# harryjfowen/PointsToWood

Hardware: AMD Instinct MI355X
Metric: classified points/sec (higher is better)
Workload: dtype f16x3

## Files before the change

include/p2w.h:

```cpp
#ifndef P2W_H
#define P2W_H

#include <stddef.h>
#include <stdint.h>

#ifdef __cplusplus
extern "C" {
#endif

typedef void* p2w_stream_t;

#define P2W_OK 0
#define P2W_EINVAL (-1)
#define P2W_ENULL (-2)
#define P2W_EALIGN (-3)
#define P2W_EWORKSPACE (-4)
#define P2W_EUNSUPPORTED (-5)

#define P2W_MAX_K 64
#define P2W_MAX_K_WIDE 100
#define P2W_MAX_K_CONV 32

int32_t p2w_version(void);
const char* p2w_strerror(int32_t code);
// ... 190 lines not shown
                    const float* sf, const int32_t* nbr, const int32_t* deg, int32_t kw, int32_t M,
                    const float* w1r4 , const float* W2p, int32_t C1, int32_t C2,
                    const float* b2, const float* bn_s, const float* bn_t, float* out, int32_t ldo,
                    p2w_stream_t stream);

#define P2W_PREC_F16X3 0
#define P2W_PREC_F16 1
#define P2W_PREC_BF16 2
int32_t p2w_packed_dims_h(int32_t prec, int32_t N, int32_t K, int32_t* N_pad, int32_t* K_pad);

#define P2W_GEMM_TILE_128 1
#define P2W_GEMM_TILE_256 2
#define P2W_GEMM_GENERIC_EPI 4
#define P2W_GEMM_ORDER_ROWS 8
#define P2W_GEMM_ORDER_COLS 16
#define P2W_GEMM_RESIDUAL_H 32
#define P2W_GEMM_STREAMK 64
#define P2W_GEMM_NO_STREAMK 128
#define P2W_GEMM_TILE_64 (1 << 24)
#define P2W_GEMM_NO_TILE_64 (1 << 25)
#define P2W_SA_ITEM_256 1
#define P2W_SA_ITEM_128 2
#define P2W_SA_PACK8 4

int32_t p2w_gemm_h2(int32_t prec, const void* A_h, int32_t ldh_a, const void* Wh, float wscale, int32_t M, int32_t N,
                    int32_t K, const p2w_epilogue* epi, float* out_f32, int32_t ldo, void* out_h, int32_t ldh_o,
                    int32_t flags, p2w_stream_t stream);
size_t p2w_gemm_h2_sk_ws_bytes(void);
int32_t p2w_gemm_h2_sk(int32_t prec, const void* A_h, int32_t ldh_a, const void* Wh, float wscale, int32_t M, int32_t N,
                       int32_t K, const p2w_epilogue* epi, float* out_f32, int32_t ldo, void* out_h, int32_t ldh_o,
                       void* ws, size_t ws_bytes, int32_t flags, p2w_stream_t stream);
size_t p2w_gemm_h2_rowdot_ws_bytes(int32_t M, int32_t N);
int32_t p2w_gemm_h2_rowdot(int32_t prec, const void* A_h, int32_t ldh_a, const void* Wh, float wscale, int32_t M, int32_t N,
                           int32_t K, const p2w_epilogue* epi, const float* dot_w, float dot_b, float* out, void* ws,
                           size_t ws_bytes, int32_t flags, p2w_stream_t stream);
size_t p2w_sa_conv_h_ws_bytes(int32_t M, int32_t flags);
int32_t p2w_sa_conv_h(int32_t prec, const float* P, int32_t ldp, int32_t n_src, const float* xyzr_src, const int32_t* idx,
                      const int32_t* batch_dst, const float* sf, const int32_t* nbr, const int32_t* deg, int32_t kw,
                      int32_t M, const float* w1r4, const void* W2h, float wscale, int32_t C1, int32_t C2,
                      const float* b2, const float* bn_s, const float* bn_t, float* out, int32_t ldo, void* out_h,
                      int32_t ldh, void* ws, size_t ws_bytes, int32_t flags, p2w_stream_t stream);
int32_t p2w_sa_conv_h_rows(int32_t prec, const float* P, int32_t ldp, int32_t n_src, const float* xyzr_src, const int32_t* idx,
                           const int32_t* batch_dst, const float* sf, const int32_t* nbr, const int32_t* deg, int32_t kw,
                           int32_t M, const float* w1r4, const void* W2h, float wscale, int32_t C1, int32_t C2,
                           const float* b2, const float* bn_s, const float* bn_t, float* out, int32_t ldo, void* out_h,
                           int32_t ldh, void* ws, size_t ws_bytes, int32_t flags, const int32_t* src_row, uint32_t* range,
// ... 132 lines not shown
```

pointstowood_amd/_lib.py:

```python
from __future__ import annotations

import ctypes as C
import os

import torch

_HERE = os.path.dirname(os.path.abspath(__file__))
LIB_PATH = os.path.join(_HERE, "libp2w_gfx950.so")

_vp, _i32, _f32, _sz = C.c_void_p, C.c_int32, C.c_float, C.c_size_t


class Epilogue(C.Structure):
    _fields_ = [("bias", _vp), ("sc0", _vp), ("sh0", _vp), ("sc1", _vp), ("sh1", _vp), ("residual", _vp),
                ("ldr", _i32), ("relu0", _i32), ("relu1", _i32), ("relu2", _i32), ("relu_final", _i32), ("range", _vp),
                ("interp", _vp), ("interp_rows", _i32)]


class BnStage(C.Structure):
    _fields_ = [("dw_w", _vp), ("dw_b", _vp), ("gamma", _vp), ("beta", _vp), ("running_mean", _vp), ("running_var", _vp),
                ("momentum", C.c_double), ("eps", C.c_double), ("relu", _i32)]


SEARCH_X_INDEX_IN_W, SEARCH_Q_ROW_IN_W, SEARCH_BOX = 1, 2, 4
PREC_F16X3, PREC_F16, PREC_BF16 = 0, 1, 2
PREC_OF = {"f16x3": PREC_F16X3, "fp16": PREC_F16, "bf16": PREC_BF16}
GEMM_TILE_128, GEMM_TILE_256, GEMM_GENERIC_EPI, GEMM_ORDER_ROWS, GEMM_ORDER_COLS, GEMM_RESIDUAL_H = 1, 2, 4, 8, 16, 32
GEMM_STREAMK, GEMM_NO_STREAMK = 64, 128
SA_ITEM_256, SA_ITEM_128, SA_PACK8 = 1, 2, 4
CLUSTER_LINK, CLUSTER_COMPRESS, CLUSTER_NUMBER, CLUSTER_ALL = 1, 2, 4, 7
MAX_K_WIDE = 100
EVAL_CHUNK, EVAL_MAX_CLASSES = 4096, 8
LOSS_CHUNK = 4096
EDGE_CHUNK = 1024
BN_GROUP = 16
BN_CHAIN_MAX, BN_CHAIN_ROWS = 3, 32
FEED_CHUNK, FEED_STREAM = 256, 0x50325746
SAMPLE_STREAM, SAMPLE_TILE, SAMPLE_N_MAX = 0x50325753, 1024, 1 << 24
F32, F16 = 0, 1

SIGNATURES = {
    "p2w_version": (_i32, []),
    "p2w_strerror": (C.c_char_p, [_i32]),
    "p2w_pack_xyzr": (_i32, [_vp, _i32, _vp, _vp, _i32, _i32, _vp, _vp, _vp]),
    "p2w_voxel_sample_ws_bytes": (_sz, [_i32]),
    "p2w_voxel_sample": (_i32, [_vp, _vp, _i32, _i32, _f32, _vp, _vp, _vp, _vp, _vp, _vp, _vp, _vp, _vp, _vp, _sz, _vp]),
    "p2w_voxel_sample_table_ws_bytes": (_sz, [_i32, C.c_int64]),
    "p2w_voxel_sample_table": (_i32, [_vp, _vp, _i32, _i32, _f32, _vp, _vp, _vp, _vp, _vp, _vp, _vp, _vp, _vp, _vp, _vp, _vp, C.c_int64,
                                      _vp, _sz, _vp]),
    "p2w_voxel_sample_table_prepare": (_i32, [_vp, _sz, _vp]),
    "p2w_voxel_sample_table_prepared": (_i32, [_vp, _vp, _i32, _i32, _f32, _vp, _vp, _vp, _vp, _vp, _vp, _vp, _vp, _vp, _vp, _vp, _vp, C.c_int64,
                                               _vp, _sz, _vp]),
# ... 189 lines not shown
```

pointstowood_amd/csrc/p2w_feat.hip:

```cpp
#include "p2w_hgemm.h"
#include "p2w_segmax.h"

constexpr int G_BM = 128, G_BN = 128, G_BK = 32, G_LD = 36;

extern "C" void p2w_packed_dims(int32_t N, int32_t K, int32_t* N_pad, int32_t* K_pad) {
    if (N_pad) *N_pad = (N + 255) / 256 * 256;
    if (K_pad) *K_pad = (K + G_BK - 1) / G_BK * G_BK;
}
extern "C" int32_t p2w_packed_dims_h(int32_t prec, int32_t N, int32_t K, int32_t* N_pad, int32_t* K_pad) {
    if (prec < P2W_PREC_F16X3 || prec > P2W_PREC_BF16) return P2W_EINVAL;
    const int ka = prec == P2W_PREC_F16X3 ? 32 : 64;
    if (N_pad) *N_pad = (N + 255) / 256 * 256;
    if (K_pad) *K_pad = (K + ka - 1) / ka * ka;
    return P2W_OK;
}

__device__ __forceinline__ void mma_slab(const float* __restrict__ As, const float* __restrict__ Bs, int wr, int wc, int lane,
                                         f32x16 (&acc)[2][2]) {
    const int r = lane & 31, h = lane >> 5;
#pragma unroll
    for (int kk = 0; kk < G_BK; kk += 8) {
        const float4 a0 = *reinterpret_cast<const float4*>(&As[(wr * 64 + r) * G_LD + kk + 4 * h]);
        const float4 a1 = *reinterpret_cast<const float4*>(&As[(wr * 64 + 32 + r) * G_LD + kk + 4 * h]);
        const float4 b0 = *reinterpret_cast<const float4*>(&Bs[(wc * 64 + r) * G_LD + kk + 4 * h]);
// ... 364 lines not shown
    EpiArgs ep = {};
    if (epi) {
        if ((epi->sc0 && !epi->sh0) || (epi->sc1 && !epi->sh1)) return P2W_ENULL;
        if (epi->residual || epi->interp) return P2W_EUNSUPPORTED;
        ep = {epi->bias, epi->sc0, epi->sh0, epi->sc1, epi->sh1, nullptr, 0, epi->relu0, epi->relu1, epi->relu2, epi->relu_final, nullptr, epi->range, nullptr};
    }
    const _Float16* Ah = static_cast<const _Float16*>(A_h);
    const _Float16* Wp = static_cast<const _Float16*>(Wh);
    const int ldpart = rowdot_ldpart(M);
    const int32_t rc = prec == P2W_PREC_F16X3
        ? launch_gemm_h<0>(Ah, ldh_a, Wp, wscale, M, N, K, ep, nullptr, 0, nullptr, 0, flags, p2w_s(stream), dot_w, part, ldpart)
        : p2w_gemm_h1_impl(prec, Ah, ldh_a, Wp, wscale, M, N, K, ep, nullptr, 0, nullptr, 0, flags, p2w_s(stream), dot_w, part, ldpart);
    if (rc != P2W_OK) return rc;
    rowdot_finish_kernel<<<p2w_cdiv(M, 256), 256, 0, p2w_s(stream)>>>(part, ldpart, (N + 63) / 64, dot_b, M, out);
    return P2W_LAUNCH_STATUS();
}

__global__ __launch_bounds__(256) void sa_edge_meta_kernel(const float4* __restrict__ xyzr, const int* __restrict__ idx,
                                                           const int* __restrict__ batch_dst, const float* __restrict__ sf,
                                                           const int* __restrict__ nbr, const int* __restrict__ deg, int kw,
                                                           int M, int n_src, int ldp4, int G, const int* __restrict__ list,
                                                           const int* __restrict__ n_list_dev, const int* __restrict__ src_row,
                                                           int* __restrict__ meta_j, float4* __restrict__ meta_g, int* __restrict__ desc,
                                                           float4* __restrict__ zero_row) {
    const long g = (long)blockIdx.x * 256 + threadIdx.x;
    if (zero_row && g < ldp4) zero_row[g] = make_float4(0.f, 0.f, 0.f, 0.f);
    const int n_groups = list ? *n_list_dev : M;
    const int gpt = 32 / G;
    const long n_tiles = ((long)n_groups + gpt - 1) / gpt;
    if (g >= n_tiles * 32) return;
    const int gi = (int)(g / G), slot = (int)(g % G);
    const int tgt = gi < n_groups ? (list ? list[gi] : gi) : -1;
    int j = 0, d = 0;
    float rx = 0.f, ry = 0.f, rz = 0.f, rf = 0.f, nrm = 0.f;
    bool valid = false;
    if (tgt >= 0) {
        d = min(deg[tgt], kw);
        const int self = idx[tgt];
        const float s = sf[batch_dst[tgt]];
        const float4 pi = xyzr[self];
        valid = slot < d;
        j = valid ? nbr[(size_t)tgt * kw + slot] : self;
        if (j < 0) j = self;
        const float4 pj = xyzr[j];
        if (valid) {
            rx = pj.x / s - pi.x / s; ry = pj.y / s - pi.y / s; rz = pj.z / s - pi.z / s;
            nrm = sqrtf(((rx * rx) + (ry * ry)) + (rz * rz));
            rf = pj.w;
        }
    }
    float dmax = nrm;
    for (int off = G >> 1; off >= 1; off >>= 1) dmax = fmaxf(dmax, __shfl_xor(dmax, off));
    const float den = dmax + 1e-8f;
    meta_j[g] = (valid ? (src_row ? src_row[j] : j) : n_src) * ldp4;
    meta_g[g] = make_float4(rx / den, ry / den, rz / den, rf);
    if (slot == 0) desc[gi] = tgt >= 0 ? ((tgt << 6) | d) : -1;
}

__global__ __launch_bounds__(SA_PART_BLOCK) void sa_part_count_kernel(const int* __restrict__ deg, int kw, int M, int* __restrict__ blk_small) {
    const int t = blockIdx.x * SA_PART_BLOCK + threadIdx.x;
    const bool small = t < M && min(deg[t], kw) <= 8;
    const int c = __syncthreads_count(small);
    if (threadIdx.x == 0) blk_small[blockIdx.x] = c;
}
__global__ __launch_bounds__(1024) void sa_part_scan_kernel(int* __restrict__ blk_small, int nblk, int M, int* __restrict__ counts) {
    __shared__ int part[1024];
    const int per = (nblk + 1023) / 1024, b0 = threadIdx.x * per, b1 = min(b0 + per, nblk);
    int sum = 0;
    for (int b = b0; b < b1; ++b) sum += blk_small[b];
    part[threadIdx.x] = sum;
    __syncthreads();
    for (int off = 1; off < 1024; off <<= 1) {
        const int v = threadIdx.x >= off ? part[threadIdx.x - off] : 0;
        __syncthreads();
        part[threadIdx.x] += v;
        __syncthreads();
    }
    int run = part[threadIdx.x] - sum;
// ... 370 lines not shown
```

pointstowood_amd/csrc/p2w_hgemm.h:

```cpp
#pragma once
#include "p2w_common.h"
#include <type_traits>

typedef float f32x16 __attribute__((ext_vector_type(16)));
typedef _Float16 h8 __attribute__((ext_vector_type(8)));
typedef __bf16 bf8 __attribute__((ext_vector_type(8)));
typedef __fp16 hpair __attribute__((ext_vector_type(2)));
typedef _Float16 hpairn __attribute__((ext_vector_type(2)));
typedef __bf16 bpair __attribute__((ext_vector_type(2)));
typedef float fpair __attribute__((ext_vector_type(2)));
typedef __attribute__((address_space(3))) void* lds_vp;
typedef const __attribute__((address_space(1))) void* glb_vp;

constexpr int H_BK = 32;
constexpr int SA_EPI_COLS = 1024;

template <int PREC> struct HCfg {
    static constexpr int planes = PREC == 0 ? 2 : 1;
    static constexpr int kslab = PREC == 0 ? 32 : 64;
    static constexpr int kalign = PREC == 0 ? 32 : 64;
};

template <int PREC>
__device__ __forceinline__ f32x16 h_mfma(h8 a, h8 b, f32x16 c) {
    if constexpr (PREC == 2)
        return __builtin_amdgcn_mfma_f32_32x32x16_bf16(__builtin_bit_cast(bf8, a), __builtin_bit_cast(bf8, b), c, 0, 0, 0);
    else
        return __builtin_amdgcn_mfma_f32_32x32x16_f16(a, b, c, 0, 0, 0);
}

typedef float f32x4 __attribute__((ext_vector_type(4)));
template <int PREC>
__device__ __forceinline__ f32x4 h_mfma16(h8 a, h8 b, f32x4 c) {
    if constexpr (PREC == 2)
        return __builtin_amdgcn_mfma_f32_16x16x32_bf16(__builtin_bit_cast(bf8, a), __builtin_bit_cast(bf8, b), c, 0, 0, 0);
    else
        return __builtin_amdgcn_mfma_f32_16x16x32_f16(a, b, c, 0, 0, 0);
}

__device__ __forceinline__ void split_pair(float a, float b, unsigned& hi, unsigned& lo) {
    const hpair h = __builtin_amdgcn_cvt_pkrtz(a, b);
    const fpair rem = {a - (float)h[0], b - (float)h[1]};
    const hpairn l = __builtin_convertvector(rem, hpairn);
    hi = __builtin_bit_cast(unsigned, h);
    lo = __builtin_bit_cast(unsigned, l);
}
template <int PREC>
__device__ __forceinline__ unsigned pack_pair(float a, float b) {
    if constexpr (PREC == 2) {
        const fpair p = {a, b};
        return __builtin_bit_cast(unsigned, __builtin_convertvector(p, bpair));
    } else {
        const fpair p = {__builtin_amdgcn_fmed3f(a, -65504.f, 65504.f), __builtin_amdgcn_fmed3f(b, -65504.f, 65504.f)};
        return __builtin_bit_cast(unsigned, __builtin_convertvector(p, hpairn));
    }
}
template <int PREC>
__device__ __forceinline__ void h_store2(_Float16* __restrict__ base, unsigned ldh, unsigned row, unsigned col, float a, float b) {
    if constexpr (PREC == 0) {
        unsigned hw, lw;
        split_pair(a, b, hw, lw);
        _Float16* p = base + (size_t)row * (2 * ldh) + 64 * (col >> 5) + (col & 31);
        *reinterpret_cast<unsigned*>(p) = hw;
        *reinterpret_cast<unsigned*>(p + 32) = lw;
    } else {
        *reinterpret_cast<unsigned*>(base + (size_t)row * ldh + col) = pack_pair<PREC>(a, b);
    }
}
// ... 806 lines not shown
#pragma unroll
                    for (int r = 0; r < 4; ++r) {
                        const int slot = r + 4 * h;
                        if (slot < d) ext = fmaxf(ext, sgn * acc[i][j][4 * q + r]);
                    }
                }
                {
                    const auto sw = __builtin_amdgcn_permlane32_swap(__float_as_uint(ext), __float_as_uint(ext), false, false);
                    ext = fmaxf(__uint_as_float(sw[0]), __uint_as_float(sw[1]));
                }
                float vmax = fmaf(fmaxf(fmaf(sgn * ext, wscale, e.bias[j]), 0.f), e.s[j], e.t[j]);
                if (d == 0 || !cv) vmax = 0.f;
                amax = nan_max(amax, fabsf(vmax));
                if (cv && h == 0 && out) out[(size_t)tgt * ldo + col] = vmax;
                if (out_h2) {
                    const float nb = __uint_as_float(__builtin_amdgcn_update_dpp(0, __float_as_uint(vmax), 0xB1, 0xf, 0xf, false));
                    if (h == 0 && (lane & 1) == 0 && col < ldh) h_store2<PREC>(out_h2, ldh, tgt, col, vmax, nb);
                }
            }
        }
    }
}

template <int PREC, int BN, int RT, int G>
__global__ __launch_bounds__(512, 2) void sa_conv16p_kernel(const float* __restrict__ P, int ldp, const int* __restrict__ meta_j,
                                                            const float4* __restrict__ meta_g, const int* __restrict__ desc,
                                                            const int* __restrict__ tiles_dev, int M, const float* __restrict__ w1r4, int C1, int C1pad,
                                                            const _Float16* __restrict__ W2h, size_t plane, float wscale, int C2,
                                                            int nMt_, int nNt, const float* __restrict__ b2,
                                                            const float* __restrict__ bn_s, const float* __restrict__ bn_t,
                                                            float* __restrict__ out, int ldo, _Float16* __restrict__ out_h2,
                                                            int ldh, unsigned* __restrict__ range) {
    constexpr int NP = HCfg<PREC>::planes;
    constexpr int WCn = BN / 64, BM = 32 * RT * (8 / WCn), NW = 8, NR = BM / 128;
    constexpr int GPT = 32 / G;
    if (tiles_dev) M = *tiles_dev;
    const int nMt = tiles_dev ? (M + BM / 32 - 1) / (BM / 32) : nMt_;
    if (M <= 0) return;
    constexpr int A_CH = 4 * NP * BM, STAGE_CH = A_CH + 4 * NP * BN;
    constexpr int NWI = 4;
    constexpr int NI = (4 * NP * BN) / 64 / NWI;
    static_assert(NI >= 1, "every issuing wave has at least one W2 DMA piece per slab");
    __shared__ __attribute__((aligned(16))) char S[2 * STAGE_CH * 16 + 4 * 512 * 4 + 3 * SA_EPI_COLS * 4];
    float* const Wr = reinterpret_cast<float*>(S + 2 * STAGE_CH * 16);
    float* const Ep = Wr + 4 * 512;
    const int tid = threadIdx.x, lane = tid & 63;
    for (int i = tid; i < 4 * C1pad; i += 512) Wr[i] = w1r4[i];
    for (int i = tid; i < C2; i += 512) { Ep[i] = b2[i]; Ep[SA_EPI_COLS + i] = bn_s[i]; Ep[2 * SA_EPI_COLS + i] = bn_t[i]; }
    const int wave = __builtin_amdgcn_readfirstlane(tid >> 6), wr = wave / WCn, wc = wave % WCn;
    const int nitems = nMt * nNt, nslab = C1pad / H_BK;
    int first, stride, limit;
    if ((gridDim.x & 7) == 0) {
        const int xcd = blockIdx.x & 7, slot = blockIdx.x >> 3, per = gridDim.x >> 3;
        const int chunk = (nitems + 7) >> 3;
        first = xcd * chunk + slot; stride = per; limit = min((xcd + 1) * chunk, nitems);
    } else {
        first = blockIdx.x; stride = gridDim.x; limit = nitems;
    }
    if (first >= limit) return;
    const int my_items = (limit - first + stride - 1) / stride;
    const int total = my_items * nslab;

    auto item_mt = [&](int it) { return (first + it * stride) / nNt; };
    auto item_nt = [&](int it) { return (first + it * stride) % nNt; };

    constexpr int RCH = 4 * NP;
    auto img = [](int row, int chunk) { return (row * RCH + (NP == 2 ? (chunk ^ ((row >> 1) & 7)) : (chunk ^ ((row >> 2) & 3)))) * 16; };
    auto imgA = [](int row, int chunk) { return (row * RCH + (NP == 2 ? (chunk ^ ((row >> 1) & 7) ^ ((row & 1) << 2)) : (chunk ^ ((row >> 2) & 3)))) * 16; };
    const int prow = tid >> 2, pq = tid & 3;
    const int a_dst = imgA(prow, pq);
    size_t boff[NI];
    int dstc[NI];
    (void)plane;
#pragma unroll
    for (int i = 0; i < NI; ++i) {
        const int g2 = (wave % NWI) + NWI * i;
        const int row = (NP == 2 ? 8 : 16) * g2 + (lane >> (NP == 2 ? 3 : 2));
        const int c = NP == 2 ? ((lane & 7) ^ ((row >> 1) & 7)) : ((lane & 3) ^ ((row >> 2) & 3));
        boff[i] = (size_t)row * (NP * C1pad) + 8 * c;
        dstc[i] = A_CH + g2 * 64;
    }
    constexpr int KADV = NP == 2 ? 2 : 1;
    auto issue = [&](int stage, const _Float16* wbase, int k0) {
        if (wave >= NWI) return;
#pragma unroll
        for (int i = 0; i < NI; ++i)
            __builtin_amdgcn_global_load_lds((glb_vp)(wbase + boff[i] + KADV * k0),
                                             (lds_vp)(S + ((size_t)stage * STAGE_CH + dstc[i]) * 16), 16, 0, 0);
    };
    struct Meta { int j[NR]; float4 g[NR]; };
    struct Vals { float4 v[NR][2]; };
    const int last_row = M * 32 - 1;
    auto load_meta = [&](int mt_, Meta& m) {
#pragma unroll
        for (int u = 0; u < NR; ++u) {
            const int row = min(mt_ * BM + prow + 128 * u, last_row);
            m.j[u] = meta_j[row];
            m.g[u] = meta_g[row];
        }
    };
    auto gather = [&](const Meta& m, int k0, Vals& dst) {
        const unsigned k4 = (unsigned)(k0 >> 2) + 2u * pq;
#pragma unroll
        for (int u = 0; u < NR; ++u) {
            const float4* p = reinterpret_cast<const float4*>(P) + ((unsigned)m.j[u] + k4);
            dst.v[u][0] = p[0];
            dst.v[u][1] = p[1];
        }
    };
    struct WRegs { float4 w[2][4]; };
    auto load_w = [&](int k0, WRegs& wr_) {
        const int k = k0 + 8 * pq;
#pragma unroll
        for (int half = 0; half < 2; ++half)
#pragma unroll
            for (int c = 0; c < 4; ++c) wr_.w[half][c] = *reinterpret_cast<const float4*>(&Wr[c * C1pad + k + 4 * half]);
    };
    const unsigned lds_base = (unsigned)(uintptr_t)(lds_vp)S;
    auto produce = [&](int stage, const Meta& m, int k0, const Vals& src, const WRegs& wr_) {
        const int k = k0 + 8 * pq;
#pragma unroll
      for (int u = 0; u < NR; ++u) {
        const float4 rg = m.g[u];
        unsigned hiw[4], low[4];
#pragma unroll
        for (int half = 0; half < 2; ++half) {
            const int kk = k + 4 * half;
            const float4 wx = wr_.w[half][0], wy = wr_.w[half][1], wz = wr_.w[half][2], wf = wr_.w[half][3];
            const float4 p = src.v[u][half];
            const float gx = rg.x, gy = rg.y, gz = rg.z, gw = rg.w;
            float v[4];
            v[0] = fmaxf(fmaf(gw, wf.x, fmaf(gz, wz.x, fmaf(gy, wy.x, fmaf(gx, wx.x, p.x)))), 0.f);
            v[1] = fmaxf(fmaf(gw, wf.y, fmaf(gz, wz.y, fmaf(gy, wy.y, fmaf(gx, wx.y, p.y)))), 0.f);
            v[2] = fmaxf(fmaf(gw, wf.z, fmaf(gz, wz.z, fmaf(gy, wy.z, fmaf(gx, wx.z, p.z)))), 0.f);
            v[3] = fmaxf(fmaf(gw, wf.w, fmaf(gz, wz.w, fmaf(gy, wy.w, fmaf(gx, wx.w, p.w)))), 0.f);
            if constexpr (PREC == 0) {
                unsigned h01, l01, h23, l23;
                split_pair(v[0], v[1], h01, l01);
                split_pair(v[2], v[3], h23, l23);
                hiw[2 * half] = h01; hiw[2 * half + 1] = h23;
                low[2 * half] = l01; low[2 * half + 1] = l23;
            } else {
                hiw[2 * half] = pack_pair<PREC>(v[0], v[1]); hiw[2 * half + 1] = pack_pair<PREC>(v[2], v[3]);
            }
        }
        const unsigned sa = lds_base + (unsigned)stage * (STAGE_CH * 16) + (unsigned)(a_dst + u * 128 * RCH * 16);
        {
            typedef unsigned u32x4 __attribute__((ext_vector_type(4)));
            const u32x4 hv = {hiw[0], hiw[1], hiw[2], hiw[3]};
            asm volatile("ds_write_b128 %0, %1" :: "v"(sa), "v"(hv) : "memory");
            if constexpr (PREC == 0) {
                const u32x4 lv = {low[0], low[1], low[2], low[3]};
                asm volatile("ds_write_b128 %0, %1" :: "v"(sa ^ 64u), "v"(lv) : "memory");
            }
        }
      }
    };

    const int r = lane & 31, h = lane >> 5;
    int offA[RT], offB[2];
#pragma unroll
    for (int t = 0; t < RT; ++t) offA[t] = imgA(wr * 32 * RT + 32 * t + r, h);
#pragma unroll
    for (int t = 0; t < 2; ++t) offB[t] = A_CH * 16 + img(wc * 64 + 32 * t + r, h);
    f32x16 acc[RT][2];
#pragma unroll
    for (int i = 0; i < RT; ++i)
#pragma unroll
        for (int j = 0; j < 2; ++j)
#pragma unroll
            for (int e = 0; e < 16; ++e) acc[i][j][e] = 0.f;

    struct Cur { int it, s, mt, nt; };
    auto nxt = [&](Cur c) {
        if (++c.s == nslab) {
            c.s = 0; ++c.it;
            const int itc = min(c.it, my_items - 1);
            c.mt = item_mt(itc); c.nt = item_nt(itc);
        }
        return c;
    };
    auto meta_of = [&](Cur c, Meta& m) { load_meta(c.mt, m); };
    auto k_of = [&](Cur c) { return (c.it < my_items ? c.s : nslab - 1) * H_BK; };
    Cur c0 = {0, 0, item_mt(0), item_nt(0)}, c1 = nxt(c0), c2 = nxt(c1), c3 = nxt(c2);
    Meta ma, mb, mc;
    Vals va;
    {
        Meta m0;
        meta_of(c0, m0);
        meta_of(c1, ma);
        meta_of(c2, mb);
        meta_of(c3, mc);
        __syncthreads();
        issue(0, W2h + (size_t)c0.nt * BN * NP * C1pad, 0);
        gather(m0, 0, va);
        WRegs w0;
        load_w(0, w0);
        produce(0, m0, 0, va, w0);
        gather(ma, k_of(c1), va);
#pragma unroll
        for (int u = 0; u < NR; ++u)
#pragma unroll
            for (int hh = 0; hh < 2; ++hh)
                asm volatile("" : "+v"(va.v[u][hh].x), "+v"(va.v[u][hh].y), "+v"(va.v[u][hh].z), "+v"(va.v[u][hh].w));
    }
    struct Degs { int d[RT][GPT]; };
    auto load_deg = [&](int mt_, Degs& e) {
#pragma unroll
        for (int i = 0; i < RT; ++i)
#pragma unroll
            for (int q = 0; q < GPT; ++q) e.d[i][q] = desc[min(mt_ * (BM / 32) + wr * RT + i, M - 1) * GPT + q];
    };
    Degs dg_;
    load_deg(c0.mt, dg_);
    float amax = 0.f;
    for (int g = 0; g < total; ++g) {
        asm volatile("" ::: "memory");
        __builtin_amdgcn_s_waitcnt(0xC07F);
        __builtin_amdgcn_s_barrier();
        asm volatile("" ::: "memory");
        Vals vb;
        gather(mb, k_of(c2), vb);
        meta_of(c3, mc);
        Degs dg_n;
        load_deg(c1.mt, dg_n);
        WRegs wk;
        load_w(k_of(c1), wk);
        __builtin_amdgcn_sched_barrier(0);
        if (g + 1 < total)
            issue((g + 1) & 1, W2h + (size_t)c1.nt * BN * NP * C1pad, c1.s * H_BK);
        const char* st = S + (size_t)(g & 1) * STAGE_CH * 16;
        h8 afq[2][NP][RT], bfq[2][NP][2];
#pragma unroll
        for (int kk = 0; kk < 2; ++kk)
#pragma unroll
            for (int p = 0; p < NP; ++p) {
#pragma unroll
                for (int t = 0; t < RT; ++t) afq[kk][p][t] = *reinterpret_cast<const h8*>(st + (offA[t] ^ (kk << 5) ^ (p << 6)));
#pragma unroll
                for (int t = 0; t < 2; ++t) bfq[kk][p][t] = *reinterpret_cast<const h8*>(st + (offB[t] ^ (kk << 5) ^ (p << 6)));
            }
#pragma unroll
        for (int kk = 0; kk < 2; ++kk) {
            auto& af = afq[kk];
            auto& bf = bfq[kk];
#pragma unroll
            for (int i = 0; i < RT; ++i)
#pragma unroll
                for (int j = 0; j < 2; ++j) {
                    if constexpr (PREC == 0) {
                        acc[i][j] = h_mfma<PREC>(af[1][i], bf[0][j], acc[i][j]);
                        acc[i][j] = h_mfma<PREC>(af[0][i], bf[1][j], acc[i][j]);
                    }
                    acc[i][j] = h_mfma<PREC>(af[0][i], bf[0][j], acc[i][j]);
                }
            if (kk == 0) {
                produce((g + 1) & 1, ma, k_of(c1), va, wk);
                constexpr int NM = 2 * RT * (PREC == 0 ? 3 : 1);
#pragma unroll
                for (int q = 0; q < NM; ++q) {
                    __builtin_amdgcn_sched_group_barrier(0x008, 1, 0);
                    __builtin_amdgcn_sched_group_barrier(0x002, (PREC == 0 ? 16 : 40) * NR / RT, 0);
                }
                __builtin_amdgcn_sched_barrier(0);
            }
        }
#pragma unroll
        for (int u = 0; u < NR; ++u) {
            asm volatile("" : "+v"(vb.v[u][0].x), "+v"(vb.v[u][0].y), "+v"(vb.v[u][0].z), "+v"(vb.v[u][0].w),
                              "+v"(vb.v[u][1].x), "+v"(vb.v[u][1].y), "+v"(vb.v[u][1].z), "+v"(vb.v[u][1].w));
            asm volatile("" : "+v"(mc.j[u]), "+v"(mc.g[u].x), "+v"(mc.g[u].y), "+v"(mc.g[u].z), "+v"(mc.g[u].w));
        }
#pragma unroll
        for (int i = 0; i < RT; ++i)
#pragma unroll
            for (int q = 0; q < GPT; ++q) asm volatile("" : "+v"(dg_n.d[i][q]));
        __builtin_amdgcn_s_waitcnt(p2w_vmcnt_imm(0));
        if (c0.s == nslab - 1) {
            SaEpiRegs<RT, GPT> e;
#pragma unroll
            for (int j = 0; j < 2; ++j) {
                const int col = min(c0.nt * BN + wc * 64 + j * 32 + (lane & 31), C2 - 1);
                e.bias[j] = Ep[col]; e.s[j] = Ep[SA_EPI_COLS + col]; e.t[j] = Ep[2 * SA_EPI_COLS + col];
            }
#pragma unroll
            for (int i = 0; i < RT; ++i)
#pragma unroll
                for (int q = 0; q < GPT; ++q) e.dsc[i][q] = (c0.mt * (BM / 32) + wr * RT + i >= M) ? -1 : dg_.d[i][q];
            sa_epilogue_regs<PREC, RT, G>(acc, wscale, c0.nt * BN, wc, lane, e, C2, out, ldo, out_h2, ldh, amax);
#pragma unroll
            for (int i = 0; i < RT; ++i)
#pragma unroll
                for (int j = 0; j < 2; ++j)
#pragma unroll
                    for (int e2 = 0; e2 < 16; ++e2) acc[i][j][e2] = 0.f;
        }
        __builtin_amdgcn_sched_barrier(0);
        va = vb; ma = mb; mb = mc; dg_ = dg_n;
        c0 = c1; c1 = c2; c2 = c3; c3 = nxt(c3);
    }
    if (range) range_commit_max(range, amax, lane);
}


__global__ __launch_bounds__(256) void sa_edge_meta_kernel(const float4* __restrict__ xyzr, const int* __restrict__ idx, const int* __restrict__ batch_dst,
                                    const float* __restrict__ sf, const int* __restrict__ nbr, const int* __restrict__ deg, int kw,
                                    int M, int n_src, int ldp4, int G, const int* __restrict__ list, const int* __restrict__ n_list_dev,
                                    const int* __restrict__ src_row, int* __restrict__ meta_j, float4* __restrict__ meta_g, int* __restrict__ desc,
                                    float4* __restrict__ zero_row);
constexpr int SA_PART_BLOCK = 1024;
__global__ __launch_bounds__(SA_PART_BLOCK) void sa_part_count_kernel(const int* __restrict__ deg, int kw, int M, int* __restrict__ blk_small);
__global__ __launch_bounds__(1024) void sa_part_scan_kernel(int* __restrict__ blk_small, int nblk, int M, int* __restrict__ counts);
__global__ __launch_bounds__(SA_PART_BLOCK) void sa_part_scatter_kernel(const int* __restrict__ deg, int kw, int M, const int* __restrict__ blk_small,
                                                                     int* __restrict__ list_small, int* __restrict__ list_large);

struct SaWs {
    float4 *mg_l, *mg_s;
    int *mj_l, *mj_s, *desc_l, *desc_s;
    int *list_s, *list_l, *blk, *counts;
    long t32, t8, nblk;
};
static inline SaWs sa_conv_carve(P2wArena& a, long M, int flags) {
    const bool pack8 = (flags & P2W_SA_PACK8) != 0;
    SaWs W = {};
    W.t32 = M;
    W.t8 = pack8 ? (M + 3) / 4 : 0;
    W.nblk = pack8 ? (M + SA_PART_BLOCK - 1) / SA_PART_BLOCK : 0;
    W.mg_l = a.take<float4>((size_t)W.t32 * 32, 16);
    W.mg_s = a.take<float4>((size_t)W.t8 * 32, 16);
    W.mj_l = a.take<int>((size_t)W.t32 * 32, 4);
    W.mj_s = a.take<int>((size_t)W.t8 * 32, 4);
    W.desc_l = a.take<int>((size_t)W.t32, 4);
    W.desc_s = a.take<int>((size_t)W.t8 * 4, 4);
    if (!pack8) { a.raw(256, 1); return W; }
    W.list_s = a.take<int>((size_t)M, 4);
    W.list_l = a.take<int>((size_t)M, 4);
    W.blk = a.take<int>((size_t)W.nblk, 4);
    W.counts = a.take<int>(16, 4);
    a.raw(1024, 1);
    return W;
}

template <int PREC>
static int32_t launch_sa_conv_h(const float* P, int32_t ldp, int32_t n_src, const float* xyzr_src, const int32_t* idx, const int32_t* batch_dst,
                                const float* sf, const int32_t* nbr, const int32_t* deg, int32_t kw, int32_t M,
                                const float* w1r4, const _Float16* W2h, float wscale, int32_t C1, int32_t C2, const float* b2,
                                const float* bn_s, const float* bn_t, float* out, int32_t ldo, _Float16* out_h2, int32_t ldh,
                                void* ws, size_t ws_bytes, int32_t flags, hipStream_t stream, const int32_t* src_row = nullptr,
                                unsigned* range = nullptr) {
    constexpr int KA = HCfg<PREC>::kalign;
    const int C2pad = (C2 + 255) / 256 * 256, C1pad = (C1 + KA - 1) / KA * KA;
    if (C1pad > 512 || C2 > SA_EPI_COLS || (long)M >= (1L << 25) || ((long)n_src + 1) * (ldp / 4) >= (1L << 31)) return P2W_EUNSUPPORTED;
    if (ldp < C1pad) return P2W_EINVAL;
    P2wArena arena(ws);
    const SaWs L = sa_conv_carve(arena, M, flags);
    if (ws == nullptr || ws_bytes < arena.bytes()) return P2W_EWORKSPACE;
    if (reinterpret_cast<uintptr_t>(ws) & 15u) return P2W_EALIGN;
    const int n_cu = p2w_cu_count();
    const bool wide = (flags & (P2W_SA_ITEM_256 | P2W_SA_ITEM_128)) ? (flags & P2W_SA_ITEM_256) != 0 : C2 > 128;
    const int tpi = wide ? 4 : 8, nNt3 = p2w_cdiv(C2, wide ? 256 : 128);
    const float4* x4 = reinterpret_cast<const float4*>(xyzr_src);
    auto run = [&](auto g_c, const int* list, const int* n_list_dev, const int* tiles_dev, long tiles_max, float4* meta_g, int* meta_j,
                   int* desc) {
        constexpr int G = decltype(g_c)::value;
        const long rows_max = tiles_max * 32;
        sa_edge_meta_kernel<<<p2w_cdiv(rows_max, 256), 256, 0, stream>>>(x4, idx, batch_dst, sf, nbr, deg, kw, M, n_src, ldp / 4, G,
                                                                       list, n_list_dev, src_row, meta_j, meta_g, desc,
                                                                       reinterpret_cast<float4*>(const_cast<float*>(P) + (size_t)n_src * ldp));
        const long items = p2w_cdiv(tiles_max, tpi) * nNt3;
        int grid = (int)(items < n_cu ? items : n_cu);
        if (grid >= 8) grid &= ~7;
        const int nMt3 = (int)p2w_cdiv(tiles_max, tpi);
        if (wide)
            sa_conv16p_kernel<PREC, 256, 2, G><<<grid, 512, 0, stream>>>(
                P, ldp, meta_j, meta_g, desc, tiles_dev, (int)tiles_max, w1r4, C1, C1pad, W2h, (size_t)C2pad * C1pad, wscale, C2, nMt3,
                nNt3, b2, bn_s, bn_t, out, ldo, out_h2, ldh, range);
        else
            sa_conv16p_kernel<PREC, 128, 2, G><<<grid, 512, 0, stream>>>(
                P, ldp, meta_j, meta_g, desc, tiles_dev, (int)tiles_max, w1r4, C1, C1pad, W2h, (size_t)C2pad * C1pad, wscale, C2, nMt3,
                nNt3, b2, bn_s, bn_t, out, ldo, out_h2, ldh, range);
    };
    if (!(flags & P2W_SA_PACK8)) {
        run(std::integral_constant<int, 32>{}, nullptr, nullptr, nullptr, M, L.mg_l, L.mj_l, L.desc_l);
        return P2W_LAUNCH_STATUS();
    }
    int* counts = L.counts;
    sa_part_count_kernel<<<(int)L.nblk, SA_PART_BLOCK, 0, stream>>>(deg, kw, M, L.blk);
    sa_part_scan_kernel<<<1, 1024, 0, stream>>>(L.blk, (int)L.nblk, M, counts);
    sa_part_scatter_kernel<<<(int)L.nblk, SA_PART_BLOCK, 0, stream>>>(deg, kw, M, L.blk, L.list_s, L.list_l);
    run(std::integral_constant<int, 8>{}, L.list_s, counts + 0, counts + 2, L.t8, L.mg_s, L.mj_s, L.desc_s);
    run(std::integral_constant<int, 32>{}, L.list_l, counts + 1, counts + 3, L.t32, L.mg_l, L.mj_l, L.desc_l);
    return P2W_LAUNCH_STATUS();
}

int32_t p2w_gemm_h1_impl(int32_t prec, const _Float16* Ah, int32_t ldh_a, const _Float16* Wp, float wscale, int32_t M, int32_t N,
                         int32_t K, const EpiArgs& ep, float* out_f32, int32_t ldo, _Float16* out_h2, int32_t ldh_o,
                         int32_t flags, hipStream_t stream, const float* dotw = nullptr, float* part = nullptr, int32_t ldpart = 0,
                         float* skws = nullptr, size_t skws_bytes = 0);
int32_t p2w_sa_conv_h1_impl(int32_t prec, const float* P, int32_t ldp, int32_t n_src, const float* xyzr_src, const int32_t* idx,
                            const int32_t* batch_dst, const float* sf, const int32_t* nbr, const int32_t* deg, int32_t kw,
                            int32_t M, const float* w1r4, const _Float16* W2h, float wscale, int32_t C1, int32_t C2,
                            const float* b2, const float* bn_s, const float* bn_t, float* out, int32_t ldo, _Float16* out_h2,
                            int32_t ldh, void* ws, size_t ws_bytes, int32_t flags, hipStream_t stream, const int32_t* src_row = nullptr,
                            unsigned* range = nullptr);
```

pointstowood_amd/engine.py:

```python
from __future__ import annotations

import contextlib
import ctypes as C
import math
from dataclasses import dataclass, field, fields

import torch

from . import _lib
from ._lib import GEMM_RESIDUAL_H, PREC_F16X3, PREC_OF, SA_PACK8, SEARCH_BOX, SEARCH_Q_ROW_IN_W, SEARCH_X_INDEX_IN_W, Epilogue, check, lib, ptr, ws_bytes

BN_EPS = 1e-5
SA_RES = (0.04, 0.08, 0.16)


@dataclass
class Linear:
    w: torch.Tensor
    N: int
    K: int
    bias: torch.Tensor | None = None
    sc0: torch.Tensor | None = None
    sh0: torch.Tensor | None = None
    sc1: torch.Tensor | None = None
# ... 43 lines not shown
                w16 = w16.contiguous().to(device)
            else:
                w16 = Ws.to(torch.float32).to(torch.float16 if precision == "fp16" else torch.bfloat16).contiguous().to(device)
            return Linear(w=None, N=N, K=K, w16=w16, wscale=2.0 ** (-e), **vec)

        self.stem_w = f32(sd["stem_mlp.0.0.weight"])
        self.stem_b = f32(sd["stem_mlp.0.0.bias"])
        self.sa = []
        f_in = C_
        for l in (1, 2, 3):
            p = f"sa{l}_module"
            W1, b1 = sd[p + ".conv.local_nn.0.0.weight"], sd[p + ".conv.local_nn.0.0.bias"]
            C1 = W1.shape[0]
            W2, b2 = sd[p + ".conv.local_nn.1.0.weight"], sd[p + ".conv.local_nn.1.0.bias"]
            C2 = W2.shape[0]
            s2, t2 = _bn_affine(sd, p + ".conv.local_nn.1.2")
            _, C1p = _lib.packed_dims(C2, C1, prec)
            w1r4 = torch.zeros((4, C1p), dtype=torch.float32)
            w1r4[:, :C1] = W1[:, f_in:f_in + 4].t()
            lvl = {
                "F_in": f_in, "C1": C1, "C2": C2,
                "hoist": pack(W1[:, :f_in], bias=b1),
                "w1r4": f32(w1r4),
                "w1r_bound": float(w1r4.abs().sum(dim=0).max()),
                "W2": pack(W2), "b2": f32(b2), "bn_s": f32(s2), "bn_t": f32(t2),
            }
            r, F, E = p + ".residual_block", C2, 4 * C2
            se, te = _bn_affine(sd, r + ".expand.1")
            dws, dwt = self._dw_affine(sd, r + ".conv.0")
            lvl["g1"] = pack(sd[r + ".expand.0.weight"][:, :, 0].double() * se[:, None],
                             bias=se * sd[r + ".expand.0.bias"].double() + te, relu0=1, sc0=dws, sh0=dwt, relu1=1)
            sp, tp = _bn_affine(sd, r + ".conv.0.pointwise_bn")
            s1, t1 = _bn_affine(sd, r + ".conv.1")
            dws2, dwt2 = self._dw_affine(sd, r + ".conv.3")
            lvl["g2"] = pack(sd[r + ".conv.0.pointwise_conv.weight"][:, :, 0].double() * sp[:, None],
                             bias=sp * sd[r + ".conv.0.pointwise_conv.bias"].double() + tp, relu0=1,
                             sc0=s1, sh0=t1, relu1=1, sc1=dws2, sh1=dwt2, relu2=1)
            sp2, tp2 = _bn_affine(sd, r + ".conv.3.pointwise_bn")
            lvl["g3"] = pack(sd[r + ".conv.3.pointwise_conv.weight"][:, :, 0].double() * sp2[:, None],
                             bias=sp2 * sd[r + ".conv.3.pointwise_conv.bias"].double() + tp2, relu0=1)
            s4, t4 = _bn_affine(sd, r + ".conv.4")
            spj, tpj = _bn_affine(sd, r + ".project.1")
            Wp = sd[r + ".project.0.weight"][:, :, 0].double()
            lvl["g4"] = pack(spj[:, None] * Wp * s4[None, :],
                             bias=spj * (Wp @ t4 + sd[r + ".project.0.bias"].double()) + tpj, relu_final=1)
            self.sa.append(lvl)
# ... 630 lines not shown
        wait = lambda ev: torch.cuda.current_stream().wait_event(ev) if ev is not None else None

        def need(table, key):
            while table.get(key) is None and geo.launch_searches is not None:
                geo.launch_searches(1)
            wait(table.get(key))

        def stage(count):
            if geo.launch_searches is not None and geo.search_stream is not None:
                ev = torch.cuda.Event()
                ev.record()
                geo.launch_searches(count, after=ev)
        if keep is not None:
            keep["stem"] = x0
        x3 = None
        for l in (1, 2, 3):
            p, src, dst = w.sa[l - 1], lv[l - 1], lv[l]
            M, C1, C2, E = dst.n, p["C1"], p["C2"], 4 * p["C2"]
            C1p = pad8(C1)
            P = early["P1"] if l == 1 else self._hoist(xh[l - 1], pitch[l - 1], src.n, p, l)
            need(geo.ev_nbr, l)
            conv = new(M, C2) if (keep is not None or not res_h) else None
            convh = newh(M, C2)
            sa_flags = self.sa_flags | (SA_PACK8 if (l == 1 and self.sa_pack) else 0)
            meta = torch.empty(int(L.p2w_sa_conv_h_ws_bytes(M, sa_flags)) + 65536, dtype=torch.uint8, device=dev)
            if keep is not None:
                keep[f"sa{l}_module.ws"] = meta
            self._call("sa_conv", L.p2w_sa_conv_h_rows, prec, ptr(P), C1p, src.n, ptr(src.xyzr), ptr(dst.idx), ptr(dst.batch),
                       ptr(geo.sf), ptr(dst.nbr), ptr(dst.deg), geo.k, M, ptr(p["w1r4"]), ptr(p["W2"].w16),
                       p["W2"].wscale, C1, C2, ptr(p["b2"]), ptr(p["bn_s"]), ptr(p["bn_t"]), ptr(conv), C2, ptr(convh),
                       pad8(C2), ptr(meta), meta.numel(), sa_flags, ptr(geo.inv0) if (l == 1 and sorted0) else None, self._watch(f"sa{l}", M))
            stage(1 if l < 3 else 2)
            out = new(M, C2) if (keep is not None or l == 3) else None
            def res_chunk(r0, m, bufs):
                e1, e2 = bufs
                self._gemm_h2("gemm_res", convh[r0:], pad8(C2), m, p["g1"], out_h2=e1, ldh_o=pad8(E), watch=f"res{l}.1")
                self._gemm_h2("gemm_res", e1, pad8(E), m, p["g2"], out_h2=e2, ldh_o=pad8(E), watch=f"res{l}.2")
                self._gemm_h2("gemm_res", e2, pad8(E), m, p["g3"], out_h2=e1, ldh_o=pad8(E), watch=f"res{l}.3")
                self._gemm_h2("gemm_res", e1, pad8(E), m, p["g4"], out_f32=None if out is None else out[r0:], ldo=C2,
                              out_h2=xh[l][r0:], ldh_o=pitch[l],
                              residual=convh[r0:] if res_h else conv[r0:], ldr=pad8(C2) if res_h else C2, residual_h=res_h,
                              watch=f"res{l}.4")
            self._chunk_chains(geo, M, E, E // 256, True, lambda rows: (newh(rows, E), newh(rows, E)), res_chunk)
            if l == 3:
                x3 = out
            if keep is not None:
                keep[f"sa{l}_module.conv"], keep[f"sa{l}_module.out"] = conv, out
# ... 266 lines not shown
```

Baseline: 20.97 million.

## Skip reflectance weight term in SA conv when all edge reflectance deltas are zero

The edge-meta kernel sets a per-call tagged device flag whenever any edge has a nonzero reflectance feature. The SA conv kernel reads that flag and, when no nonzero value was seen and the weights are finite, runs a 3-column variant that drops the fourth FMA and its weight loads. The change also swaps the f16x3 hi/lo split for a v_fma_mix-based version and simplifies the LDS destination indexing. It adds an atomic tag counter, a workspace word per run and a duplicated pipeline instantiation that increases code size.

```diff
diff --git a/include/p2w.h b/include/p2w.h
--- a/include/p2w.h
+++ b/include/p2w.h
@@ -236,6 +236,8 @@
 #define P2W_SA_ITEM_256 1
 #define P2W_SA_ITEM_128 2
 #define P2W_SA_PACK8 4
+#define P2W_SA_REFL_W_FINITE 8
+#define P2W_SA_NO_XYZ_FAST 16
 
 int32_t p2w_gemm_h2(int32_t prec, const void* A_h, int32_t ldh_a, const void* Wh, float wscale, int32_t M, int32_t N,
                     int32_t K, const p2w_epilogue* epi, float* out_f32, int32_t ldo, void* out_h, int32_t ldh_o,
diff --git a/pointstowood_amd/_lib.py b/pointstowood_amd/_lib.py
--- a/pointstowood_amd/_lib.py
+++ b/pointstowood_amd/_lib.py
@@ -27,7 +27,12 @@
 PREC_OF = {"f16x3": PREC_F16X3, "fp16": PREC_F16, "bf16": PREC_BF16}
 GEMM_TILE_128, GEMM_TILE_256, GEMM_GENERIC_EPI, GEMM_ORDER_ROWS, GEMM_ORDER_COLS, GEMM_RESIDUAL_H = 1, 2, 4, 8, 16, 32
 GEMM_STREAMK, GEMM_NO_STREAMK = 64, 128
-SA_ITEM_256, SA_ITEM_128, SA_PACK8 = 1, 2, 4
+SA_ITEM_256, SA_ITEM_128, SA_PACK8, SA_REFL_W_FINITE, SA_NO_XYZ_FAST = 1, 2, 4, 8, 16
+
+
+def sa_weight_flags(w1r4) -> int:
+    import torch
+    return SA_REFL_W_FINITE if bool(torch.isfinite(w1r4[3]).all()) else 0
 CLUSTER_LINK, CLUSTER_COMPRESS, CLUSTER_NUMBER, CLUSTER_ALL = 1, 2, 4, 7
 MAX_K_WIDE = 100
 EVAL_CHUNK, EVAL_MAX_CLASSES = 4096, 8
diff --git a/pointstowood_amd/csrc/p2w_feat.hip b/pointstowood_amd/csrc/p2w_feat.hip
--- a/pointstowood_amd/csrc/p2w_feat.hip
+++ b/pointstowood_amd/csrc/p2w_feat.hip
@@ -410,7 +410,8 @@
                                                            int M, int n_src, int ldp4, int G, const int* __restrict__ list,
                                                            const int* __restrict__ n_list_dev, const int* __restrict__ src_row,
                                                            int* __restrict__ meta_j, float4* __restrict__ meta_g, int* __restrict__ desc,
-                                                           float4* __restrict__ zero_row) {
+                                                           float4* __restrict__ zero_row, unsigned* __restrict__ refl_word,
+                                                           unsigned refl_tag) {
     const long g = (long)blockIdx.x * 256 + threadIdx.x;
     if (zero_row && g < ldp4) zero_row[g] = make_float4(0.f, 0.f, 0.f, 0.f);
     const int n_groups = list ? *n_list_dev : M;
@@ -442,6 +443,7 @@
     const float den = dmax + 1e-8f;
     meta_j[g] = (valid ? (src_row ? src_row[j] : j) : n_src) * ldp4;
     meta_g[g] = make_float4(rx / den, ry / den, rz / den, rf);
+    if (refl_word && __float_as_uint(rf) != 0u) *refl_word = refl_tag;
     if (slot == 0) desc[gi] = tgt >= 0 ? ((tgt << 6) | d) : -1;
 }
 
diff --git a/pointstowood_amd/csrc/p2w_hgemm.h b/pointstowood_amd/csrc/p2w_hgemm.h
--- a/pointstowood_amd/csrc/p2w_hgemm.h
+++ b/pointstowood_amd/csrc/p2w_hgemm.h
@@ -1,5 +1,6 @@
 #pragma once
 #include "p2w_common.h"
+#include <atomic>
 #include <type_traits>
 
 typedef float f32x16 __attribute__((ext_vector_type(16)));
@@ -44,6 +45,15 @@
     const hpairn l = __builtin_convertvector(rem, hpairn);
     hi = __builtin_bit_cast(unsigned, h);
     lo = __builtin_bit_cast(unsigned, l);
+}
+__device__ __forceinline__ void split_pair_mix(float a, float b, unsigned& hi, unsigned& lo) {
+    const hpair h = __builtin_amdgcn_cvt_pkrtz(a, b);
+    hi = __builtin_bit_cast(unsigned, h);
+    float ra, rb;
+    asm("v_fma_mix_f32 %0, %1, -1.0, %2 op_sel_hi:[1,0,0]" : "=v"(ra) : "v"(hi), "v"(a));
+    asm("v_fma_mix_f32 %0, %1, -1.0, %2 op_sel:[1,0,0] op_sel_hi:[1,0,0]" : "=v"(rb) : "v"(hi), "v"(b));
+    const fpair rem = {ra, rb};
+    lo = __builtin_bit_cast(unsigned, __builtin_convertvector(rem, hpairn));
 }
 template <int PREC>
 __device__ __forceinline__ unsigned pack_pair(float a, float b) {
@@ -896,6 +906,7 @@
     }
 }
 
+template <int NC> struct SaWRegs { static constexpr int nc = NC; float4 w[2][NC]; };
 template <int PREC, int BN, int RT, int G>
 __global__ __launch_bounds__(512, 2) void sa_conv16p_kernel(const float* __restrict__ P, int ldp, const int* __restrict__ meta_j,
                                                             const float4* __restrict__ meta_g, const int* __restrict__ desc,
@@ -904,7 +915,8 @@
                                                             int nMt_, int nNt, const float* __restrict__ b2,
                                                             const float* __restrict__ bn_s, const float* __restrict__ bn_t,
                                                             float* __restrict__ out, int ldo, _Float16* __restrict__ out_h2,
-                                                            int ldh, unsigned* __restrict__ range) {
+                                                            int ldh, unsigned* __restrict__ range,
+                                                            const unsigned* __restrict__ refl_word, unsigned refl_tag) {
     constexpr int NP = HCfg<PREC>::planes;
     constexpr int WCn = BN / 64, BM = 32 * RT * (8 / WCn), NW = 8, NR = BM / 128;
     constexpr int GPT = 32 / G;
@@ -944,7 +956,7 @@
     const int prow = tid >> 2, pq = tid & 3;
     const int a_dst = imgA(prow, pq);
     size_t boff[NI];
-    int dstc[NI];
+    const int dst0 = A_CH + (wave % NWI) * 64;
     (void)plane;
 #pragma unroll
     for (int i = 0; i < NI; ++i) {
@@ -952,7 +964,6 @@
         const int row = (NP == 2 ? 8 : 16) * g2 + (lane >> (NP == 2 ? 3 : 2));
         const int c = NP == 2 ? ((lane & 7) ^ ((row >> 1) & 7)) : ((lane & 3) ^ ((row >> 2) & 3));
         boff[i] = (size_t)row * (NP * C1pad) + 8 * c;
-        dstc[i] = A_CH + g2 * 64;
     }
     constexpr int KADV = NP == 2 ? 2 : 1;
     auto issue = [&](int stage, const _Float16* wbase, int k0) {
@@ -960,7 +971,7 @@
 #pragma unroll
         for (int i = 0; i < NI; ++i)
             __builtin_amdgcn_global_load_lds((glb_vp)(wbase + boff[i] + KADV * k0),
-                                             (lds_vp)(S + ((size_t)stage * STAGE_CH + dstc[i]) * 16), 16, 0, 0);
+                                             (lds_vp)(S + ((size_t)stage * STAGE_CH + dst0 + NWI * 64 * i) * 16), 16, 0, 0);
     };
     struct Meta { int j[NR]; float4 g[NR]; };
     struct Vals { float4 v[NR][2]; };
@@ -982,16 +993,17 @@
             dst.v[u][1] = p[1];
         }
     };
-    struct WRegs { float4 w[2][4]; };
-    auto load_w = [&](int k0, WRegs& wr_) {
+    auto load_w = [&](int k0, auto& wr_) {
+        constexpr int NC = std::remove_reference_t<decltype(wr_)>::nc;
         const int k = k0 + 8 * pq;
 #pragma unroll
         for (int half = 0; half < 2; ++half)
 #pragma unroll
-            for (int c = 0; c < 4; ++c) wr_.w[half][c] = *reinterpret_cast<const float4*>(&Wr[c * C1pad + k + 4 * half]);
+            for (int c = 0; c < NC; ++c) wr_.w[half][c] = *reinterpret_cast<const float4*>(&Wr[c * C1pad + k + 4 * half]);
     };
     const unsigned lds_base = (unsigned)(uintptr_t)(lds_vp)S;
-    auto produce = [&](int stage, const Meta& m, int k0, const Vals& src, const WRegs& wr_) {
+    auto produce = [&](int stage, const Meta& m, int k0, const Vals& src, const auto& wr_) {
+        constexpr int NC = std::remove_reference_t<decltype(wr_)>::nc;
         const int k = k0 + 8 * pq;
 #pragma unroll
       for (int u = 0; u < NR; ++u) {
@@ -1000,18 +1012,25 @@
 #pragma unroll
         for (int half = 0; half < 2; ++half) {
             const int kk = k + 4 * half;
-            const float4 wx = wr_.w[half][0], wy = wr_.w[half][1], wz = wr_.w[half][2], wf = wr_.w[half][3];
+            const float4 wx = wr_.w[half][0], wy = wr_.w[half][1], wz = wr_.w[half][2];
             const float4 p = src.v[u][half];
-            const float gx = rg.x, gy = rg.y, gz = rg.z, gw = rg.w;
+            const float gx = rg.x, gy = rg.y, gz = rg.z;
             float v[4];
-            v[0] = fmaxf(fmaf(gw, wf.x, fmaf(gz, wz.x, fmaf(gy, wy.x, fmaf(gx, wx.x, p.x)))), 0.f);
-            v[1] = fmaxf(fmaf(gw, wf.y, fmaf(gz, wz.y, fmaf(gy, wy.y, fmaf(gx, wx.y, p.y)))), 0.f);
-            v[2] = fmaxf(fmaf(gw, wf.z, fmaf(gz, wz.z, fmaf(gy, wy.z, fmaf(gx, wx.z, p.z)))), 0.f);
-            v[3] = fmaxf(fmaf(gw, wf.w, fmaf(gz, wz.w, fmaf(gy, wy.w, fmaf(gx, wx.w, p.w)))), 0.f);
+            v[0] = fmaf(gz, wz.x, fmaf(gy, wy.x, fmaf(gx, wx.x, p.x)));
+            v[1] = fmaf(gz, wz.y, fmaf(gy, wy.y, fmaf(gx, wx.y, p.y)));
+            v[2] = fmaf(gz, wz.z, fmaf(gy, wy.z, fmaf(gx, wx.z, p.z)));
+            v[3] = fmaf(gz, wz.w, fmaf(gy, wy.w, fmaf(gx, wx.w, p.w)));
+            if constexpr (NC == 4) {
+                const float4 wf = wr_.w[half][3];
+                const float gw = rg.w;
+                v[0] = fmaf(gw, wf.x, v[0]); v[1] = fmaf(gw, wf.y, v[1]); v[2] = fmaf(gw, wf.z, v[2]); v[3] = fmaf(gw, wf.w, v[3]);
+            }
+#pragma unroll
+            for (int e = 0; e < 4; ++e) v[e] = fmaxf(v[e], 0.f);
             if constexpr (PREC == 0) {
                 unsigned h01, l01, h23, l23;
-                split_pair(v[0], v[1], h01, l01);
-                split_pair(v[2], v[3], h23, l23);
+                split_pair_mix(v[0], v[1], h01, l01);
+                split_pair_mix(v[2], v[3], h23, l23);
                 hiw[2 * half] = h01; hiw[2 * half + 1] = h23;
                 low[2 * half] = l01; low[2 * half + 1] = l23;
             } else {
@@ -1056,6 +1075,9 @@
     };
     auto meta_of = [&](Cur c, Meta& m) { load_meta(c.mt, m); };
     auto k_of = [&](Cur c) { return (c.it < my_items ? c.s : nslab - 1) * H_BK; };
+    float amax = 0.f;
+    auto pipeline = [&](auto w_c) __attribute__((always_inline)) {
+    using WRegs = decltype(w_c);
     Cur c0 = {0, 0, item_mt(0), item_nt(0)}, c1 = nxt(c0), c2 = nxt(c1), c3 = nxt(c2);
     Meta ma, mb, mc;
     Vals va;
@@ -1087,7 +1109,6 @@
     };
     Degs dg_;
     load_deg(c0.mt, dg_);
-    float amax = 0.f;
     for (int g = 0; g < total; ++g) {
         asm volatile("" ::: "memory");
         __builtin_amdgcn_s_waitcnt(0xC07F);
@@ -1134,7 +1155,7 @@
 #pragma unroll
                 for (int q = 0; q < NM; ++q) {
                     __builtin_amdgcn_sched_group_barrier(0x008, 1, 0);
-                    __builtin_amdgcn_sched_group_barrier(0x002, (PREC == 0 ? 16 : 40) * NR / RT, 0);
+                    __builtin_amdgcn_sched_group_barrier(0x002, (PREC == 0 ? (WRegs::nc == 3 ? 12 : 16) : 40) * NR / RT, 0);
                 }
                 __builtin_amdgcn_sched_barrier(0);
             }
@@ -1173,6 +1194,9 @@
         va = vb; ma = mb; mb = mc; dg_ = dg_n;
         c0 = c1; c1 = c2; c2 = c3; c3 = nxt(c3);
     }
+    };
+    if (refl_word && (unsigned)__builtin_amdgcn_readfirstlane((int)*refl_word) != refl_tag) pipeline(SaWRegs<3>{});
+    else pipeline(SaWRegs<4>{});
     if (range) range_commit_max(range, amax, lane);
 }
 
@@ -1181,7 +1205,7 @@
                                     const float* __restrict__ sf, const int* __restrict__ nbr, const int* __restrict__ deg, int kw,
                                     int M, int n_src, int ldp4, int G, const int* __restrict__ list, const int* __restrict__ n_list_dev,
                                     const int* __restrict__ src_row, int* __restrict__ meta_j, float4* __restrict__ meta_g, int* __restrict__ desc,
-                                    float4* __restrict__ zero_row);
+                                    float4* __restrict__ zero_row, unsigned* __restrict__ refl_word, unsigned refl_tag);
 constexpr int SA_PART_BLOCK = 1024;
 __global__ __launch_bounds__(SA_PART_BLOCK) void sa_part_count_kernel(const int* __restrict__ deg, int kw, int M, int* __restrict__ blk_small);
 __global__ __launch_bounds__(1024) void sa_part_scan_kernel(int* __restrict__ blk_small, int nblk, int M, int* __restrict__ counts);
@@ -1193,7 +1217,9 @@
     int *mj_l, *mj_s, *desc_l, *desc_s;
     int *list_s, *list_l, *blk, *counts;
     long t32, t8, nblk;
+    unsigned* refl;
 };
+inline std::atomic<unsigned> g_sa_refl_tag{0};
 static inline SaWs sa_conv_carve(P2wArena& a, long M, int flags) {
     const bool pack8 = (flags & P2W_SA_PACK8) != 0;
     SaWs W = {};
@@ -1206,11 +1232,12 @@
     W.mj_s = a.take<int>((size_t)W.t8 * 32, 4);
     W.desc_l = a.take<int>((size_t)W.t32, 4);
     W.desc_s = a.take<int>((size_t)W.t8 * 4, 4);
-    if (!pack8) { a.raw(256, 1); return W; }
+    if (!pack8) { W.refl = a.take<unsigned>(2, 4); a.raw(248, 1); return W; }
     W.list_s = a.take<int>((size_t)M, 4);
     W.list_l = a.take<int>((size_t)M, 4);
     W.blk = a.take<int>((size_t)W.nblk, 4);
-    W.counts = a.take<int>(16, 4);
+    W.counts = a.take<int>(8, 4);
+    W.refl = a.take<unsigned>(8, 4);
     a.raw(1024, 1);
     return W;
 }
@@ -1234,13 +1261,17 @@
     const bool wide = (flags & (P2W_SA_ITEM_256 | P2W_SA_ITEM_128)) ? (flags & P2W_SA_ITEM_256) != 0 : C2 > 128;
     const int tpi = wide ? 4 : 8, nNt3 = p2w_cdiv(C2, wide ? 256 : 128);
     const float4* x4 = reinterpret_cast<const float4*>(xyzr_src);
+    const bool xyz_ok = (flags & P2W_SA_REFL_W_FINITE) && !(flags & P2W_SA_NO_XYZ_FAST);
+    const unsigned tag = g_sa_refl_tag.fetch_add(1u, std::memory_order_relaxed) + 1u;
     auto run = [&](auto g_c, const int* list, const int* n_list_dev, const int* tiles_dev, long tiles_max, float4* meta_g, int* meta_j,
-                   int* desc) {
+                   int* desc, unsigned* refl) {
+        if (!xyz_ok) refl = nullptr;
         constexpr int G = decltype(g_c)::value;
         const long rows_max = tiles_max * 32;
         sa_edge_meta_kernel<<<p2w_cdiv(rows_max, 256), 256, 0, stream>>>(x4, idx, batch_dst, sf, nbr, deg, kw, M, n_src, ldp / 4, G,
                                                                        list, n_list_dev, src_row, meta_j, meta_g, desc,
-                                                                       reinterpret_cast<float4*>(const_cast<float*>(P) + (size_t)n_src * ldp));
+                                                                       reinterpret_cast<float4*>(const_cast<float*>(P) + (size_t)n_src * ldp),
+                                                                       refl, tag);
         const long items = p2w_cdiv(tiles_max, tpi) * nNt3;
         int grid = (int)(items < n_cu ? items : n_cu);
         if (grid >= 8) grid &= ~7;
@@ -1248,22 +1279,22 @@
         if (wide)
             sa_conv16p_kernel<PREC, 256, 2, G><<<grid, 512, 0, stream>>>(
                 P, ldp, meta_j, meta_g, desc, tiles_dev, (int)tiles_max, w1r4, C1, C1pad, W2h, (size_t)C2pad * C1pad, wscale, C2, nMt3,
-                nNt3, b2, bn_s, bn_t, out, ldo, out_h2, ldh, range);
+                nNt3, b2, bn_s, bn_t, out, ldo, out_h2, ldh, range, refl, tag);
         else
             sa_conv16p_kernel<PREC, 128, 2, G><<<grid, 512, 0, stream>>>(
                 P, ldp, meta_j, meta_g, desc, tiles_dev, (int)tiles_max, w1r4, C1, C1pad, W2h, (size_t)C2pad * C1pad, wscale, C2, nMt3,
-                nNt3, b2, bn_s, bn_t, out, ldo, out_h2, ldh, range);
+                nNt3, b2, bn_s, bn_t, out, ldo, out_h2, ldh, range, refl, tag);
     };
     if (!(flags & P2W_SA_PACK8)) {
-        run(std::integral_constant<int, 32>{}, nullptr, nullptr, nullptr, M, L.mg_l, L.mj_l, L.desc_l);
+        run(std::integral_constant<int, 32>{}, nullptr, nullptr, nullptr, M, L.mg_l, L.mj_l, L.desc_l, L.refl);
         return P2W_LAUNCH_STATUS();
     }
     int* counts = L.counts;
     sa_part_count_kernel<<<(int)L.nblk, SA_PART_BLOCK, 0, stream>>>(deg, kw, M, L.blk);
     sa_part_scan_kernel<<<1, 1024, 0, stream>>>(L.blk, (int)L.nblk, M, counts);
     sa_part_scatter_kernel<<<(int)L.nblk, SA_PART_BLOCK, 0, stream>>>(deg, kw, M, L.blk, L.list_s, L.list_l);
-    run(std::integral_constant<int, 8>{}, L.list_s, counts + 0, counts + 2, L.t8, L.mg_s, L.mj_s, L.desc_s);
-    run(std::integral_constant<int, 32>{}, L.list_l, counts + 1, counts + 3, L.t32, L.mg_l, L.mj_l, L.desc_l);
+    run(std::integral_constant<int, 8>{}, L.list_s, counts + 0, counts + 2, L.t8, L.mg_s, L.mj_s, L.desc_s, L.refl + 1);
+    run(std::integral_constant<int, 32>{}, L.list_l, counts + 1, counts + 3, L.t32, L.mg_l, L.mj_l, L.desc_l, L.refl);
     return P2W_LAUNCH_STATUS();
 }
 
diff --git a/pointstowood_amd/engine.py b/pointstowood_amd/engine.py
--- a/pointstowood_amd/engine.py
+++ b/pointstowood_amd/engine.py
@@ -89,6 +89,7 @@
                 "F_in": f_in, "C1": C1, "C2": C2,
                 "hoist": pack(W1[:, :f_in], bias=b1),
                 "w1r4": f32(w1r4),
+                "sa_flags": _lib.sa_weight_flags(w1r4),
                 "w1r_bound": float(w1r4.abs().sum(dim=0).max()),
                 "W2": pack(W2), "b2": f32(b2), "bn_s": f32(s2), "bn_t": f32(t2),
             }
@@ -765,7 +766,7 @@
             need(geo.ev_nbr, l)
             conv = new(M, C2) if (keep is not None or not res_h) else None
             convh = newh(M, C2)
-            sa_flags = self.sa_flags | (SA_PACK8 if (l == 1 and self.sa_pack) else 0)
+            sa_flags = self.sa_flags | p["sa_flags"] | (SA_PACK8 if (l == 1 and self.sa_pack) else 0)
             meta = torch.empty(int(L.p2w_sa_conv_h_ws_bytes(M, sa_flags)) + 65536, dtype=torch.uint8, device=dev)
             if keep is not None:
                 keep[f"sa{l}_module.ws"] = meta
```

New measurement: 21.04 million (median of 5 runs). About the same (+0.3%).
